# JzHuai0108/sim3opt

Measured on NVIDIA B200. Metric: Sim3 LM iterations/s, higher is better.
Workload: dtype f64

## Files before the change

sim3opt_b200/csrc/amg.cu:

```cuda
#include <algorithm>
#include <cstdlib>
#include <functional>

#include <cooperative_groups.h>

#include "amg.h"
#include "comm.h"
#include "problem.h"
#include "reduce.cuh"
#include "sim3_math.cuh"

namespace s3o {

namespace {

#define DD (D * D)
constexpr int NREL = 13;
constexpr int kCoarsestMax = 16;
constexpr int kCoarsestMaxBig = 128;
constexpr int kBigGraph = 20000;
constexpr int kMaxLevels = 12;
constexpr double kOmega = 0.7;

struct LevelDev {
// ... 1523 lines not shown
        auto kgrid = [](int n) { int g = (n + 15) / 16; return g > 148 * 8 ? 148 * 8 : (g < 1 ? 1 : g); };
        std::function<void(int)> solve;
        auto cycle = [&](int l, const double *rin, double *xout) {
            LevelDev &L = st->lev[l];
            LevelDev &C = st->lev[l + 1];
            amg_row_kernel<D, 0><<<rows(L.n), 128, 0, s>>>(L.n, L.rowptr, L.colidx, L.A, L.Dinv, rin, nullptr, L.x, kOmega, sc, chk);
            amg_row_kernel<D, 1><<<rows(L.n), 128, 0, s>>>(L.n, L.rowptr, L.colidx, L.A, L.Dinv, rin, L.x, L.t, kOmega, sc, chk);
            amg_restrict_kernel<D><<<(C.n + 15) / 16, 128, 0, s>>>(C.n, C.mem_ptr, C.mem_idx, C.rel, C.pad_fine, L.t, C.r, sc, chk);
            launches += 3;
            trace_mark(p, "lev: sweep+residual+restrict");
            solve(l + 1);
            amg_prolong_kernel<D><<<(L.n + 127) / 128, 128, 0, s>>>(L.n, C.agg, C.rel, C.pad_fine, C.x2, L.x, sc, chk);
            amg_row_kernel<D, 2><<<rows(L.n), 128, 0, s>>>(L.n, L.rowptr, L.colidx, L.A, L.Dinv, rin, L.x, xout, kOmega, sc, chk);
            launches += 2;
            trace_mark(p, "lev: prolong+sweep");
        };
        solve = [&](int l) {
            LevelDev &L = st->lev[l];
            if (l >= st->coop_first) {
                CoopParams P{};
                P.nlev = nl - l;
                P.dense = st->dense ? 1 : 0;
                P.N = st->lev.back().n * D;
                P.inv = st->d_dense;
                P.kdepth = nk > l ? nk - l : 0;
                P.kmask = st->kmask >> l;
                P.dots = st->d_cdots;
                static long long *d_dbg = nullptr;
                static int dbg_calls = 0;
                static const bool dbg_on = getenv("S3O_COOP_DBG") != nullptr;
                if (dbg_on && !d_dbg) { cudaMalloc(&d_dbg, 128 * sizeof(long long)); }
                const bool dbg_now = dbg_on && ++dbg_calls == 200;
                if (dbg_now) { cudaMemsetAsync(d_dbg, 0, 128 * sizeof(long long), s); P.dbg = d_dbg; }
                for (int k = l; k < nl; ++k) {
                    LevelDev &S = st->lev[k];
                    CoopLevel &T = P.lev[k - l];
                    T.n = S.n; T.pad_fine = S.pad_fine;
                    T.rowptr = S.rowptr; T.colidx = S.colidx; T.mem_ptr = S.mem_ptr; T.mem_idx = S.mem_idx; T.agg = S.agg;
                    T.A = S.A; T.Dinv = S.Dinv; T.rel = S.rel; T.r = S.r; T.x = S.x; T.x2 = S.x2; T.t = S.t;
                    T.z1 = S.z1; T.q1 = S.q1; T.rp = S.rp; T.z2 = S.z2; T.acol = S.acol;
                }
                double omega = kOmega;
                int chk_ = chk;
                GridBarrier gb{};
                void *args[] = { &P, &omega, (void *)&sc, &chk_, &gb };
                int grid = (L.n * 8 + kCoopThreads - 1) / kCoopThreads;
                grid = std::max(8, std::min(grid, st->coop_grid));
                for (int k = 0; k < P.nlev; ++k) {
                    const long long lanes = (long long)grid * kCoopThreads, n = P.lev[k].n;
                    P.lev[k].G = n * 32 <= lanes ? 4 : (n * 16 <= lanes ? 2 : 1);
                }
                if (launch_persistent(p, (const void *)amg_coop_kernel<D>, grid, kCoopThreads, args, 5)) rc_inner = S3O_ERR_CUDA;
                ++launches;
                trace_mark(p, "cooperative kernel");
                if (dbg_now) {
                    long long h[128];
                    cudaStreamSynchronize(s);
                    cudaMemcpy(h, d_dbg, sizeof h, cudaMemcpyDeviceToHost);
                    int khz = 1; cudaDeviceGetAttribute(&khz, cudaDevAttrClockRate, p->device);
                    fprintf(stderr, "S3O_COOP_DBG: phase times of one cooperative-kernel call (us, SM clock %d kHz)\n ", khz);
                    for (int q = 1; q < 120 && h[q]; ++q) fprintf(stderr, " %d:%.1f", q, (double)(h[q] - h[q - 1]) / khz * 1e3);
                    fprintf(stderr, "\n");
                }
                return;
            }
            if ((st->kmask >> l) & 1u) {
                KScal *ks = st->d_ks + l;
                const int n = L.n * D;
                cycle(l, L.r, L.z1);
                amg_kdots_kernel<D, 128><<<kgrid(L.n), 128, 0, s>>>(L.n, L.rowptr, L.colidx, L.A, L.z1, L.r, nullptr, L.q1, p->d_partials, ks, 0, p->d_sc, chk);
                amg_kaxpy_kernel<<<std::min((n + 255) / 256, 148 * 8), 256, 0, s>>>(n, L.r, L.q1, L.rp, ks, 0, sc, chk);
                trace_mark(p, "lev: kdots+axpy");
                cycle(l, L.rp, L.z2);
                amg_kdots_kernel<D, 128><<<kgrid(L.n), 128, 0, s>>>(L.n, L.rowptr, L.colidx, L.A, L.z2, L.rp, L.q1, nullptr, p->d_partials, ks, 1, p->d_sc, chk);
                amg_kaxpy_kernel<<<std::min((n + 255) / 256, 148 * 8), 256, 0, s>>>(n, L.z1, L.z2, L.x2, ks, 1, sc, chk);
                launches += 4;
                trace_mark(p, "lev: kdots+combine");
            } else {
                cycle(l, L.r, L.x2);
            }
        };
        solve(0);
        if (rc_inner) { set_error("multilevel K-cycle: persistent-kernel launch failed: %s", s3o_last_error()); return rc_inner; }
        std::swap(st->lev[0].x, st->lev[0].x2);
    } else {
        for (int l = 0; l < lt; ++l) {
            LevelDev &L = st->lev[l];
            LevelDev &C = st->lev[l + 1];
            amg_row_kernel<D, 0><<<rows(L.n), 128, 0, s>>>(L.n, L.rowptr, L.colidx, L.A, L.Dinv, L.r, nullptr, L.x, kOmega, sc, chk);
            amg_row_kernel<D, 1><<<rows(L.n), 128, 0, s>>>(L.n, L.rowptr, L.colidx, L.A, L.Dinv, L.r, L.x, L.t, kOmega, sc, chk);
            amg_restrict_kernel<D><<<(C.n + 15) / 16, 128, 0, s>>>(C.n, C.mem_ptr, C.mem_idx, C.rel, C.pad_fine, L.t, C.r, sc, chk);
            launches += 3;
        }
        {
            TailParams P{};
            P.nlev = nl - lt;
            P.dense = st->dense ? 1 : 0;
            P.N = st->lev.back().n * D;
            P.inv = st->d_dense;
            for (int l = lt; l < nl; ++l) {
                LevelDev &L = st->lev[l];
                TailLevel &T = P.lev[l - lt];
                T.n = L.n; T.pad_fine = L.pad_fine;
                T.rowptr = L.rowptr; T.colidx = L.colidx; T.mem_ptr = L.mem_ptr; T.mem_idx = L.mem_idx; T.agg = L.agg;
                T.A = L.A; T.Dinv = L.Dinv; T.rel = L.rel; T.r = L.r; T.x = L.x; T.x2 = L.x2; T.t = L.t;
            }
            amg_tail_kernel<D><<<kTailCtas, kTailThreads, 0, s>>>(P, kOmega, sc, chk);
            for (int l = lt; l < nl; ++l) std::swap(st->lev[l].x, st->lev[l].x2);
            ++launches;
        }
        for (int l = lt - 1; l >= 0; --l) {
            LevelDev &L = st->lev[l];
            LevelDev &C = st->lev[l + 1];
            amg_prolong_kernel<D><<<(L.n + 127) / 128, 128, 0, s>>>(L.n, C.agg, C.rel, C.pad_fine, C.x, L.x, sc, chk);
            amg_row_kernel<D, 2><<<rows(L.n), 128, 0, s>>>(L.n, L.rowptr, L.colidx, L.A, L.Dinv, L.r, L.x, L.x2, kOmega, sc, chk);
            std::swap(L.x, L.x2);
            launches += 2;
        }
    }
    {
        LevelDev &L = st->lev[0];
        constexpr int NT = 256;
        const int rows = st->dist ? st->n_own : L.n_fine;
        int grid = (rows + NT - 1) / NT;
        if (grid > 148 * 8) grid = 148 * 8;
        if (grid < 1) grid = 1;
        int dgrid = (L.n * D + NT - 1) / NT;
        if (dgrid > 148) dgrid = 148;
        if (dgrid < 1) dgrid = 1;
        amg_coarse_dot_kernel<NT><<<dgrid, NT, 0, s>>>(L.n * D, L.r, L.x, p->d_partials, p->d_sc, init, tol, max_iter);
        amg_prolong0_kernel<D, NT><<<grid, NT, 0, s>>>(rows, L.agg, L.rel, L.pad_fine, L.x, p->d_z, p->d_p, sc, init);
        launches += 2;
        trace_mark(p, "coarse dot + fine prolong");
    }
    return check_launch(p, launches);
}

}

#define S3O_AMG_DISPATCH(CALL7, CALL4, CALL1)                  \
    switch (p->kind) {                                         \
    case S3O_KIND_SIM3: return CALL7;                          \
    case S3O_KIND_SCALE_TRANS: return CALL4;                   \
    case S3O_KIND_SCALE: return CALL1;                         \
    default: set_error("multilevel preconditioner: pose-graph problems only"); return S3O_ERR_UNSUPPORTED; \
    }
int amg_update_frames(s3o_problem *p) {
    S3O_AMG_DISPATCH((update_frames_t<7, S3O_KIND_SIM3>(p)), (update_frames_t<4, S3O_KIND_SCALE_TRANS>(p)),
                     (update_frames_t<1, S3O_KIND_SCALE>(p)))
}
int amg_update_values(s3o_problem *p, double lambda) {
    S3O_AMG_DISPATCH((update_values_t<7, S3O_KIND_SIM3>(p, lambda)), (update_values_t<4, S3O_KIND_SCALE_TRANS>(p, lambda)),
                     (update_values_t<1, S3O_KIND_SCALE>(p, lambda)))
}
int amg_apply(s3o_problem *p, int init, double tol, int max_iter) {
    S3O_AMG_DISPATCH(apply_t<7>(p, init, tol, max_iter), apply_t<4>(p, init, tol, max_iter), apply_t<1>(p, init, tol, max_iter))
}
#undef S3O_AMG_DISPATCH

void amg_counts(const s3o_problem *p, int64_t *rebuilds, int64_t *reuses) {
    if (!rebuilds || !reuses) { if (p->amg) p->amg->rebuilds = p->amg->reuses = 0; return; }
    *rebuilds = p->amg ? p->amg->rebuilds : 0;
    *reuses = p->amg ? p->amg->reuses : 0;
}
void amg_set_counts(s3o_problem *p, int64_t rebuilds, int64_t reuses) {
    if (p->amg) { p->amg->rebuilds = rebuilds; p->amg->reuses = reuses; }
}
void amg_invalidate_frames(s3o_problem *p) { if (p->amg) { p->amg->frames_valid = false; p->amg->lin_changed = true; } }

}
```

sim3opt_b200/csrc/kernels.cuh:

```cuda
#pragma once
#include <cuda_runtime.h>
#include <stdint.h>

namespace s3o {

struct DevScalars {
    double rz;
    double rz_new;
    double rr;
    double pq;
    double alpha, beta;
    double rr0;
    double tol2;
    double chi2;
    double scale;
    double maxdiag;
    double xmax;
    int done;
    int iters, max_iter;
    int precond_fail;
    int halo_fail;
    unsigned counters[8];
};

struct GraphDev {
    int kind, d, est_dim, ninfo;
    int nv, nv_pad, ne, ne_pad, nf, nb;
    const double *est;
    const double *aux;
    const int32_t *hidx;
    const int32_t *sv0, *sv1;
    const double *meas;
    const double *info;
    bool info_diag;
    int robust_kind;
    double robust_param;
    bool math_corrected;
    int model_flags;
    const uint8_t *primary;
    const int32_t *ghidx;
};

struct StructDev {
    const int32_t *rowptr, *colidx, *blk_row;
    const int32_t *blk_ebeg, *blk_eend;
    const int32_t *blk_src;
    const int32_t *multi_blk;
    int n_multi;
    const int32_t *colT_ptr, *colT_blk;
    const int32_t *inc_ptr, *inc_ent;
    const int32_t *e_blk;
    const int32_t *tile_row;
    int ntiles;
    int n_own;
    double *const *ghost_src;
};

constexpr int kMaxPartials = 4096;

void launch_pack_vertices(const double *aos, int n, int n_pad, int dim, double *soa, cudaStream_t st);
void launch_unpack_vertices(const double *soa, int n, int n_pad, int dim, double *aos, cudaStream_t st);
void launch_pack_edges(const double *meas_aos, const double *info_aos, const int32_t *perm, int ne, int ne_pad,
                       int est_dim, int d, int info_diag, double *meas, double *info, cudaStream_t st);

void launch_chi2(const GraphDev &g, double *partials, DevScalars *sc, cudaStream_t st);
void launch_edge_errors(const GraphDev &g, double *err_sorted , double *chi2_sorted ,
                        cudaStream_t st);
void launch_linearize(const GraphDev &g, int jac_mode, double h, double *scratch , const int32_t *e_blk,
                      const int32_t *blk_src, double *Hdirect, cudaStream_t st);
int scratch_stride(int d);
void launch_assemble(const GraphDev &g, const StructDev &s, const double *scratch, double *H, double *b,
                     cudaStream_t st);
void launch_retract(const GraphDev &g, const double *x, double *est_out, cudaStream_t st);

void launch_maxdiag(int d, const double *H, const int32_t *rowptr, int nf, double *partials, DevScalars *sc,
                    cudaStream_t st);
void launch_pcg_fin_init(DevScalars *sc, double tol, int max_iter, cudaStream_t st);
void launch_pcg_fin_spmv(DevScalars *sc, cudaStream_t st);
void launch_pcg_fin_update(DevScalars *sc, cudaStream_t st);
void launch_pack_rows(int d, const double *vec, const int32_t *idx, int n, double *out, const DevScalars *sc,
                      cudaStream_t st);
void launch_precond(int d, const double *H, const int32_t *rowptr, int nf, double lambda, double *Minv,
                    DevScalars *sc, cudaStream_t st);
void launch_spmv(int d, const double *H, const StructDev &s, int nf, double lambda, const double *p, double *q1,
                 double *T, double *partials, DevScalars *sc, int pcg_mode, cudaStream_t st);
void launch_finish_q(int d, const StructDev &s, int nf, const double *q1, const double *T, double *q, cudaStream_t st);
void launch_pcg_init(int d, int nf, const double *b, const double *Minv, double *x, double *r, double *z, double *p,
                     double *partials, DevScalars *sc, double tol, int max_iter, int dist, cudaStream_t st);
void launch_pcg_update(int d, const StructDev &s, int nf, const double *q1, const double *T, const double *Minv,
                       const double *p, double *x, double *r, double *z, double *partials, DevScalars *sc,
                       int dist, cudaStream_t st);
void launch_pcg_pupdate(int d, int nf, const double *z, double *p, const DevScalars *sc, cudaStream_t st);
void launch_scale(int n, const double *x, const double *b, double lambda, double *partials, DevScalars *sc,
                  cudaStream_t st);
int launches_per_pcg_iter();
void launch_halo_signal(long long *own_flag, long long epoch, cudaStream_t st);
void launch_halo_wait(long long *const *peer_flags, int n_peers, long long epoch, DevScalars *sc, cudaStream_t st);
void launch_scale_vec(int n, const double *in, double s, double *out, cudaStream_t st);
void launch_fill_const(int n, double v, double *out, cudaStream_t st);
void launch_fill_alternating(int n, double *out, cudaStream_t st);
int spmv_tile_blocks(int d);
int spmv2_configure();
int spmv3_tile_blocks(int d);
void launch_spmv3(int d, const double *H, const StructDev &s, int nf, double lambda, const double *p, double *q1,
// ... 10 lines not shown
```

sim3opt_b200/csrc/problem.cu:

```cuda
#include <algorithm>
#include <cfloat>
#include <cmath>
#include <cstdarg>
#include <cstdio>
#include <cstring>
#include <cstdlib>
#include <memory>
#include <thread>
#include <vector>

#include "problem.h"
#include "amg.h"
#include "direct.h"

namespace s3o {

static thread_local char g_err[512] = "";
void set_error(const char *fmt, ...) {
    va_list ap;
    va_start(ap, fmt);
    vsnprintf(g_err, sizeof g_err, fmt, ap);
    va_end(ap);
}

// ... 139 lines not shown
        launch_spmv2(p->d, p->d_H, s, own_rows(p), lambda, x, p->d_q1, p->d_T, p->d_partials, p->d_sc, pcg_mode,
                     p->dist, p->stream);
}

int do_chi2(s3o_problem *p, int which) {
    if (p->kind == S3O_KIND_BA) return ba_chi2(p, which);
    if (p->S.ne_act == 0) {
        S3O_CUDA(cudaMemsetAsync(&p->d_sc->chi2, 0, sizeof(double), p->stream));
        return allreduce_sum(p, &p->d_sc->chi2, 1);
    }
    launch_chi2(graph_view(p, which), p->d_partials, p->d_sc, p->stream);
    int rc = check_launch(p, 1);
    return rc ? rc : allreduce_sum(p, &p->d_sc->chi2, 1);
}

int do_linearize(s3o_problem *p) {
    if (p->kind == S3O_KIND_BA) return ba_linearize(p);
    const GraphDev g = graph_view(p, p->cur);
    launch_linearize(g, p->jac_mode, p->jac_h, p->d_scratch, p->d_e_blk, p->d_blk_src, p->d_H, p->stream);
    launch_assemble(g, struct_view(p), p->d_scratch, p->d_H, p->d_b, p->stream);
    amg_invalidate_frames(p);
    direct_invalidate(p);
    p->linearized = true;
    return check_launch(p, 2);
}

}

namespace s3o {
bool wants_multilevel(const s3o_problem *p) {
    const int nf = p->dist ? p->plan.nf_global : p->S.nf;
    return p->kind != S3O_KIND_BA && p->kind != 100  &&
           p->scale_model == S3O_SCALE_MODEL_DIFFERENCE &&
           (p->precond == S3O_PRECOND_MULTILEVEL || (p->precond == S3O_PRECOND_AUTO && (nf >= 20000 || p->auto_multilevel)));
}

int do_solve(s3o_problem *p, double lambda, int *status, int *iters, double *rel_res, bool defer_sync) {
    if (p->linsolver != S3O_LINSOLVER_PCG) {
        int rcd = p->dist ? S3O_OK : direct_setup(p);
        if (rcd) return rcd;
        if (direct_available(p)) {
            if ((rcd = direct_solve(p, lambda, p->reuse_factor))) return rcd;
            if (status) *status = 0;
            if (iters) *iters = 0;
            if (rel_res) *rel_res = 0;
            if (defer_sync) return S3O_OK;
            if ((rcd = sync_scalars(p))) return rcd;
            if (status) *status = p->h_sc->done;
            return S3O_OK;
        }
        if (p->linsolver == S3O_LINSOLVER_DIRECT) {
            set_error("s3o_set_linear_solver(DIRECT): %s", p->dist ? "not available in the partitioned solve"
                                                                   : "the factor of this graph is too large; use PCG");
            return S3O_ERR_UNSUPPORTED;
        }
    }
    bool amg = false;
    int rc;
    if (wants_multilevel(p)) {
        if ((rc = amg_setup(p))) return rc;
        amg = amg_levels(p) > 0;
    }
    if ((rc = pcg_prepare(p, lambda, amg))) return rc;
    if ((rc = pcg_iterate(p, lambda, amg, p->pcg_tol, p->pcg_max_iter))) return rc;
    if (p->precond == S3O_PRECOND_AUTO && (p->kind == S3O_KIND_SIM3 || p->kind == S3O_KIND_SCALE_TRANS)) {
        if (!amg && p->h_sc->iters > 256) p->auto_multilevel = true;
        else if (amg && p->auto_multilevel && p->h_sc->iters <= 8) p->auto_multilevel = false;
    }
    if (status) *status = p->h_sc->done ? p->h_sc->done : 2;
    if (iters) *iters = p->h_sc->iters;
    if (rel_res) *rel_res = p->h_sc->rr0 > 0 ? std::sqrt(p->h_sc->rr / p->h_sc->rr0) : 0.0;
    return S3O_OK;
}

void hessian_product(s3o_problem *p, const double *x) { run_spmv(p, struct_view(p), 0.0, x, 0); }

int pcg_prepare(s3o_problem *p, double lambda, bool amg) {
    launch_precond(p->d, p->d_H, p->d_rowptr, own_rows(p), lambda, p->d_Minv, p->d_sc, p->stream);
    int rc = check_launch(p, 1);
    if (!rc && amg) rc = amg_update_values(p, lambda);
    return rc;
}

int pcg_iterate(s3o_problem *p, double lambda, bool amg, double tol, int max_iter) {
    const int nf = own_rows(p), d = p->d;
    const int dist = p->dist ? 1 : 0;
    const StructDev s = struct_view(p);
    const PartitionPlan &P = p->plan;
    auto halo = [&]() -> int {
        if (!dist) return S3O_OK;
        if (p->p2p) {
            ++p->halo_epoch;
            launch_halo_signal(p->d_flag, p->halo_epoch, p->stream);
            launch_halo_wait(p->d_peer_flags, p->n_peers, p->halo_epoch, p->d_sc, p->stream);
            p->stats.kernel_launches += 2;
            return S3O_OK;
        }
        launch_pack_rows(d, p->d_p, p->d_send_idx, (int)P.send_idx.size(), p->d_sendbuf, p->d_sc, p->stream);
        p->stats.kernel_launches += 1;
        if (comm_halo(p->comm, p->d_sendbuf, P.send_off.data(), P.send_count.data(), p->d_p + (size_t)P.n_own * d,
                      P.recv_off.data(), P.recv_count.data(), d, p->stream)) {
            set_error("%s", comm_last_error());
            return S3O_ERR_NCCL;
        }
        return S3O_OK;
    };
    int rc;
    const int defer = dist || amg;
    launch_pcg_init(d, nf, p->d_b, p->d_Minv, p->d_x, p->d_r, p->d_z, p->d_p, p->d_partials, p->d_sc, tol,
                    max_iter, defer, p->stream);
    rc = check_launch(p, 1);
    if (rc) return rc;
    if (amg) {
        if ((rc = amg_apply(p, 1, tol, max_iter))) return rc;
    } else if (dist) {
        if ((rc = allreduce_sum(p, &p->d_sc->rz_new, 2))) return rc;
        launch_pcg_fin_init(p->d_sc, tol, max_iter, p->stream);
        p->stats.kernel_launches += 1;
    }
    int batch = p->last_pcg_iters > 0 ? std::max(2, std::min(64, p->last_pcg_iters - 1)) : 8, launched = 0;
    if (p->trace_state == 1 && p->trace_solve > 0) --p->trace_solve;
    for (;;) {
        for (int k = 0; k < batch; ++k) {
            const bool sample = ((launched + k) & 15) == 7 && p->spmv_ev_used < s3o_problem::kSpmvEvents;
            if (p->trace_state == 1 && p->trace_solve == 0 && launched + k == 4) { p->trace_state = 2; trace_mark(p, "start"); }
            if ((rc = halo())) return rc;
            if (sample) {
                p->spmv_ev_iter[p->spmv_ev_used] = launched + k;
                cudaEventRecord(p->spmv_ev[2 * p->spmv_ev_used], p->stream);
            }
            run_spmv(p, s, lambda, p->d_p, 1);
            trace_mark(p, "spmv");
            if (sample) cudaEventRecord(p->spmv_ev[2 * p->spmv_ev_used++ + 1], p->stream);
            if (dist) {
                if ((rc = allreduce_sum(p, &p->d_sc->pq, 1))) return rc;
                launch_pcg_fin_spmv(p->d_sc, p->stream);
            }
            launch_pcg_update(d, s, nf, p->d_q1, p->d_T, p->d_Minv, p->d_p, p->d_x, p->d_r, p->d_z, p->d_partials,
                              p->d_sc, defer, p->stream);
            trace_mark(p, "pcg_update");
            if (amg) {
                if ((rc = amg_apply(p, 0, tol, max_iter))) return rc;
                if (p->trace_state == 2) { trace_mark(p, "end"); p->trace_state = 3; }
                continue;
            }
            if (dist) {
                if ((rc = allreduce_sum(p, &p->d_sc->rz_new, 2))) return rc;
                launch_pcg_fin_update(p->d_sc, p->stream);
            }
            launch_pcg_pupdate(d, nf, p->d_z, p->d_p, p->d_sc, p->stream);
        }
        launched += batch;
        rc = check_launch(p, (amg ? (dist ? 3 : 2) : (dist ? 5 : 3)) * batch);
        if (rc) return rc;
        rc = sync_scalars(p);
        if (rc) return rc;
        if (p->trace_state == 3) {
            float tot = 0;
            cudaEventElapsedTime(&tot, p->trace.front().second, p->trace.back().second);
            fprintf(stderr, "S3O_TRACE one PCG iteration: %.1f us\n", tot * 1e3f);
            for (size_t t = 1; t < p->trace.size(); ++t) {
                float ms = 0;
                cudaEventElapsedTime(&ms, p->trace[t - 1].second, p->trace[t].second);
                fprintf(stderr, "  %-28s %8.1f us\n", p->trace[t].first, ms * 1e3f);
            }
            for (auto &t : p->trace) cudaEventDestroy(t.second);
            p->trace.clear();
            p->trace_state = 0;
        }
        for (int e = 0; e < p->spmv_ev_used; ++e) {
            float ms = 0;
            if (cudaEventElapsedTime(&ms, p->spmv_ev[2 * e], p->spmv_ev[2 * e + 1]) == cudaSuccess &&
                (!p->h_sc->done || p->spmv_ev_iter[e] < p->h_sc->iters)) {
                p->stats.ms_spmv_sampled += ms;
                p->stats.n_spmv_sampled += 1;
            }
        }
        p->spmv_ev_used = 0;
        if (p->h_sc->done || launched >= max_iter + batch) break;
        batch = launched < 16 ? std::max(2, launched / 2) : std::min(64, launched);
    }
    p->stats.pcg_iterations += p->h_sc->iters;
    p->last_pcg_iters = p->h_sc->iters;
    if (p->h_sc->done != 1) p->stats.pcg_unconverged += 1;
    return S3O_OK;
}
}

namespace s3o {

int upload_structure_arrays(s3o_problem *p, int rows_own, bool on_device) {
    HostStructure &S = p->S;
    int rc = 0;
    if (!on_device) {
        std::vector<int32_t> blk_row(S.nb);
        for (int r = 0; r < S.nf; ++r)
            for (int k = S.rowptr[r]; k < S.rowptr[r + 1]; ++k) blk_row[k] = r;
        rc = rc ? rc : upload(p, &p->d_rowptr, S.rowptr);
        rc = rc ? rc : upload(p, &p->d_colidx, S.colidx);
        rc = rc ? rc : upload(p, &p->d_blk_row, blk_row);
        rc = rc ? rc : upload(p, &p->d_colT_ptr, S.colT_ptr);
        rc = rc ? rc : upload(p, &p->d_colT_blk, S.colT_blk);
    }
    S.max_row_blocks = 0;
    for (int r = 0; r < rows_own; ++r) S.max_row_blocks = std::max(S.max_row_blocks, S.rowptr[r + 1] - S.rowptr[r]);
    S.tile_blocks = (p->spmv_version == 4 && p->d == 7) ? spmv4_tile_blocks(p->spmv4_cfg)
                    : (p->spmv_version >= 3 ? spmv3_tile_blocks(p->d) : spmv_tile_blocks(p->d));
    build_tiles(S.rowptr, rows_own, S.tile_blocks, S.tile_row);
    rc = rc ? rc : upload(p, &p->d_tile_row, S.tile_row);
    return rc;
}

int alloc_linear_system(s3o_problem *p) {
    const HostStructure &S = p->S;
    const size_t nfd = (size_t)std::max(S.nf, p->dist ? p->plan.seg : 0) * p->d, dd = (size_t)p->d * p->d;
    int rc = 0;
    rc = rc ? rc : dev_alloc(&p->d_H, (size_t)S.nb * dd + 2);
    rc = rc ? rc : dev_alloc(&p->d_b, nfd);
    rc = rc ? rc : dev_alloc(&p->d_x, nfd);
    rc = rc ? rc : dev_alloc(&p->d_r, nfd);
    rc = rc ? rc : dev_alloc(&p->d_z, nfd);
    rc = rc ? rc : dev_alloc(&p->d_p, nfd);
    rc = rc ? rc : dev_alloc(&p->d_q1, nfd);
    rc = rc ? rc : dev_alloc(&p->d_T, (size_t)S.nb * p->d);
    rc = rc ? rc : dev_alloc(&p->d_Minv, (size_t)S.nf * dd);
    return rc;
}

}

namespace {
int setup_p2p(s3o_problem *p) {
    p->want_p2p_setup = false;
    if (getenv("S3O_NO_P2P") || !uses_spmv4(p)) return S3O_OK;
    const PartitionPlan &P = p->plan;
    const int world = P.world, rank = P.rank, d = p->d;
    struct Handles { cudaIpcMemHandle_t vec, flag; };
    int rc = dev_alloc(&p->d_flag, 1);
    if (rc) return rc;
    S3O_CUDA(cudaMemsetAsync(p->d_flag, 0, sizeof(long long), p->stream));
    Handles mine{};
    int ok = cudaIpcGetMemHandle(&mine.vec, p->d_p) == cudaSuccess && cudaIpcGetMemHandle(&mine.flag, p->d_flag) == cudaSuccess;
    cudaGetLastError();
    unsigned char *d_h = nullptr;
    if ((rc = dev_alloc(&d_h, sizeof(Handles) * (size_t)(world + 1)))) return rc;
    S3O_CUDA(cudaMemcpyAsync(d_h + sizeof(Handles) * world, &mine, sizeof(Handles), cudaMemcpyHostToDevice, p->stream));
    if (comm_allgather_bytes(p->comm, d_h + sizeof(Handles) * world, d_h, sizeof(Handles), p->stream)) {
        cudaFree(d_h); set_error("%s", comm_last_error()); return S3O_ERR_NCCL;
    }
    std::vector<Handles> all(world);
    S3O_CUDA(cudaMemcpyAsync(all.data(), d_h, sizeof(Handles) * world, cudaMemcpyDeviceToHost, p->stream));
    S3O_CUDA(cudaStreamSynchronize(p->stream));
    cudaFree(d_h);
    std::vector<double *> peer_vec(world, nullptr);
    std::vector<long long *> flags;
    for (int q = 0; q < world && ok; ++q) {
        if (q == rank || P.recv_count[q] == 0) continue;
        void *v = nullptr, *f = nullptr;
        if (cudaIpcOpenMemHandle(&v, all[q].vec, cudaIpcMemLazyEnablePeerAccess) != cudaSuccess) { ok = 0; break; }
        p->ipc_mapped.push_back(v);
        if (cudaIpcOpenMemHandle(&f, all[q].flag, cudaIpcMemLazyEnablePeerAccess) != cudaSuccess) { ok = 0; break; }
        p->ipc_mapped.push_back(f);
        peer_vec[q] = (double *)v;
// ... 3 lines not shown
    if (flags.size() > 32) ok = 0;
    double *d_ok = nullptr;
    if ((rc = dev_alloc(&d_ok, 1))) return rc;
    const double fail = ok ? 0.0 : 1.0;
    S3O_CUDA(cudaMemcpyAsync(d_ok, &fail, sizeof(double), cudaMemcpyHostToDevice, p->stream));
    if (comm_allreduce_max(p->comm, d_ok, 1, p->stream)) { cudaFree(d_ok); set_error("%s", comm_last_error()); return S3O_ERR_NCCL; }
    double any_fail = 1;
    S3O_CUDA(cudaMemcpyAsync(&any_fail, d_ok, sizeof(double), cudaMemcpyDeviceToHost, p->stream));
    S3O_CUDA(cudaStreamSynchronize(p->stream));
    cudaFree(d_ok);
    if (any_fail != 0.0) { close_p2p(p); return S3O_OK; }
    std::vector<double *> src(P.n_ghost);
    for (int t = 0; t < P.n_ghost; ++t) {
        const int gidx = P.ghosts[t], q = gidx / P.seg;
        src[t] = peer_vec[q] + (size_t)(gidx - q * P.seg) * d;
    }
    rc = upload(p, &p->d_ghost_src, src);
    rc = rc ? rc : upload(p, &p->d_peer_flags, flags);
    if (rc) return rc;
    S3O_CUDA(cudaStreamSynchronize(p->stream));
    p->n_peers = (int)flags.size();
    p->halo_epoch = 0;
    p->p2p = true;
    return S3O_OK;
}
}

extern "C" {

const char *s3o_last_error(void) { return g_err; }
int s3o_version(void) { return 100; }

int s3o_device_count(void) {
    int n = 0;
    if (cudaGetDeviceCount(&n) != cudaSuccess) { cudaGetLastError(); return 0; }
    return n;
}

static constexpr int kKindLinear = 100;

static int create_impl(int kind, int linear_dim, int device, s3o_problem **out) {
    if (!out) { set_error("s3o_create: out is NULL"); return S3O_ERR_INVALID; }
    *out = nullptr;
    int d, est_dim;
    switch (kind) {
    case kKindLinear: d = linear_dim; est_dim = 0; break;
    case S3O_KIND_SIM3: d = 7; est_dim = 8; break;
    case S3O_KIND_SCALE_TRANS: d = 4; est_dim = 4; break;
    case S3O_KIND_SCALE: d = 1; est_dim = 1; break;
    case S3O_KIND_BA: d = 6; est_dim = 7; break;
    default: set_error("s3o_create: unsupported kind %d", kind); return S3O_ERR_UNSUPPORTED;
    }
    int ndev = 0;
    if (cudaGetDeviceCount(&ndev) != cudaSuccess || ndev == 0) {
        cudaGetLastError();
        set_error("s3o_create: no CUDA device available (this library has no CPU path)");
        return S3O_ERR_CUDA;
    }
    if (device < 0 || device >= ndev) { set_error("s3o_create: device %d out of range (%d devices)", device, ndev); return S3O_ERR_INVALID; }
    S3O_CUDA(cudaSetDevice(device));
    s3o_problem *p = new s3o_problem();
    p->kind = kind; p->d = d; p->est_dim = est_dim; p->ninfo = d * (d + 1) / 2; p->device = device;
    cudaError_t e = cudaStreamCreateWithFlags(&p->stream, cudaStreamNonBlocking);
    if (e != cudaSuccess) { set_error("cudaStreamCreate: %s", cudaGetErrorString(e)); delete p; return S3O_ERR_CUDA; }
    p->own_stream = true;
    if (spmv2_configure() != 0) { set_error("s3o_create: cannot configure SpMV shared memory"); delete p; return S3O_ERR_CUDA; }
    if (const char *v = getenv("S3O_TRACE")) { p->trace_state = atoi(v) > 0 ? 1 : 0; p->trace_solve = atoi(v); }
    if (const char *v = getenv("S3O_SPMV_VERSION")) p->spmv_version = atoi(v);
    if (const char *v = getenv("S3O_SPMV_GRID")) {
        const int g = atoi(v);
        if (g >= 1 && g <= kMaxPartials) p->spmv_grid_cap = g;
    }
    if (const char *v = getenv("S3O_SPMV4_CFG")) {
        const int c = atoi(v);
        if (c >= 0 && c <= 2) p->spmv4_cfg = c;
    }
    if (const char *v = getenv("S3O_PRECOND")) {
        const int k = atoi(v);
        if (k >= S3O_PRECOND_AUTO && k <= S3O_PRECOND_MULTILEVEL && (k != S3O_PRECOND_MULTILEVEL || kind != S3O_KIND_BA)) p->precond = k;
    }
    for (auto &ev : p->ev) cudaEventCreate(&ev);
    for (auto &ev : p->spmv_ev) cudaEventCreate(&ev);
    if (const char *v = getenv("S3O_COOP_LAUNCH")) p->coop_launch = atoi(v) != 0;
    if (dev_alloc(&p->d_sc, 1) || dev_alloc(&p->d_partials, 3 * kMaxPartials) || dev_alloc(&p->d_gridbar, 2) ||
        cudaMallocHost((void **)&p->h_sc, sizeof(DevScalars)) != cudaSuccess) {
        s3o_destroy(p);
        return S3O_ERR_CUDA;
    }
    cudaMemsetAsync(p->d_sc, 0, sizeof(DevScalars), p->stream);
    cudaMemsetAsync(p->d_gridbar, 0, 2 * sizeof(unsigned), p->stream);
    memset(p->h_sc, 0, sizeof(DevScalars));
    p->stats.dim = d;
    *out = p;
    return S3O_OK;
}

int s3o_create(int kind, int device, s3o_problem **out) {
    if (kind == kKindLinear) { set_error("s3o_create: unsupported kind %d", kind); return S3O_ERR_UNSUPPORTED; }
    return create_impl(kind, 0, device, out);
}

int s3o_linsolver_create(int device, int block_dim, s3o_linsolver **out) {
    if (block_dim != 1 && block_dim != 4 && block_dim != 6 && block_dim != 7) {
        set_error("s3o_linsolver_create: block dimension %d (supported: 1, 4, 6, 7)", block_dim);
        return S3O_ERR_UNSUPPORTED;
    }
    return create_impl(kKindLinear, block_dim, device, out);
}

int s3o_linsolver_destroy(s3o_linsolver *p) { return s3o_destroy(p); }

int s3o_linsolver_solve(s3o_linsolver *p, int n, const int32_t *colptr, const int32_t *rowidx, const double *blocks,
                        int column_major, double lambda, const double *b, double *x, int *method, int *pcg_iterations) {
    if (!p || p->kind != kKindLinear || n < 0 || !colptr || (n > 0 && (!rowidx || !blocks || !b || !x))) { set_error("s3o_linsolver_solve: bad arguments"); return S3O_ERR_INVALID; }
    if (n == 0) return S3O_OK;
    cudaSetDevice(p->device);
    const int d = p->d, dd = d * d, nb = colptr[n];
    bool same = p->built && p->S.nf == n && p->S.nb == nb &&
                memcmp(p->S.ccs_colptr.data(), colptr, sizeof(int32_t) * (n + 1)) == 0 &&
                memcmp(p->S.ccs_rowidx.data(), rowidx, sizeof(int32_t) * nb) == 0;
    if (!same) {
        free_structure(p);
        std::vector<int32_t> v0, v1;
        for (int c = 0; c < n; ++c) {
            bool diag = false;
            for (int k = colptr[c]; k < colptr[c + 1]; ++k) {
                const int r = rowidx[k];
                if (r < 0 || r > c || (k > colptr[c] && r <= rowidx[k - 1])) {
                    set_error("s3o_linsolver_solve: column %d is not an upper block-CCS column (rows ascending, row <= column)", c);
                    return S3O_ERR_INVALID;
                }
                if (r == c) diag = true;
                else { v0.push_back(r); v1.push_back(c); }
            }
            if (!diag) { set_error("s3o_linsolver_solve: column %d has no diagonal block", c); return S3O_ERR_INVALID; }
        }
        p->nv = n;
        p->fixed.assign(n, 0);
        build_structure_host(n, nullptr, (int)v0.size(), v0.data(), v1.data(), p->S);
        if (p->S.nb != nb || memcmp(p->S.ccs_rowidx.data(), rowidx, sizeof(int32_t) * nb) != 0) { set_error("s3o_linsolver_solve: pattern mismatch"); return S3O_ERR_INVALID; }
        int rc = upload_structure_arrays(p, n);
        rc = rc ? rc : alloc_linear_system(p);
        if (rc) { free_structure(p); return rc; }
        p->built = true;
        p->stats.n_free = n; p->stats.n_blocks = nb;
    }
    std::vector<double> H((size_t)nb * dd);
    for (int c = 0; c < nb; ++c) {
        double *dst = H.data() + (size_t)p->S.ccs2bsr[c] * dd;
        const double *src = blocks + (size_t)c * dd;
        if (!column_major) memcpy(dst, src, sizeof(double) * dd);
        else
            for (int r = 0; r < d; ++r)
                for (int cc = 0; cc < d; ++cc) dst[r * d + cc] = src[cc * d + r];
    }
    S3O_CUDA(cudaMemcpyAsync(p->d_H, H.data(), H.size() * sizeof(double), cudaMemcpyHostToDevice, p->stream));
    S3O_CUDA(cudaMemcpyAsync(p->d_b, b, (size_t)n * d * sizeof(double), cudaMemcpyHostToDevice, p->stream));
    p->stats.h2d_bytes += (int64_t)((H.size() + (size_t)n * d) * sizeof(double));
    p->linearized = true;
    direct_invalidate(p);
    int status = 0, iters = 0;
    int rc = do_solve(p, lambda, &status, &iters, nullptr);
    if (rc) return rc;
    S3O_CUDA(cudaMemcpyAsync(x, p->d_x, (size_t)n * d * sizeof(double), cudaMemcpyDeviceToHost, p->stream));
    S3O_CUDA(cudaStreamSynchronize(p->stream));
    p->stats.d2h_bytes += (int64_t)n * d * 8;
    if (method) *method = direct_available(p) && p->linsolver != S3O_LINSOLVER_PCG ? S3O_LINSOLVER_DIRECT : S3O_LINSOLVER_PCG;
    if (pcg_iterations) *pcg_iterations = iters;
    if (status == 3) { set_error("s3o_linsolver_solve: the matrix is not positive definite (pivot / PCG breakdown)"); return S3O_ERR_SOLVE; }
    if (status == 2) { set_error("s3o_linsolver_solve: PCG hit the iteration cap"); return S3O_ERR_SOLVE; }
    return S3O_OK;
}

int s3o_destroy(s3o_problem *p) {
    if (!p) return S3O_OK;
    cudaSetDevice(p->device);
    if (p->stream) cudaStreamSynchronize(p->stream);
    free_structure(p);
    ba_destroy(p);
    dev_free(p->d_meas_aos); dev_free(p->d_info_aos);
    dev_free(p->d_est[0]); dev_free(p->d_est[1]); dev_free(p->d_aux);
    dev_free(p->d_sc); dev_free(p->d_partials); dev_free(p->d_gridbar);
    comm_destroy(p->comm);
    if (p->h_sc) cudaFreeHost(p->h_sc);
    for (auto &ev : p->ev) if (ev) cudaEventDestroy(ev);
    for (auto &ev : p->spmv_ev) if (ev) cudaEventDestroy(ev);
    dev_free(p->d_est_snap);
    dev_free(p->d_stage);
    if (p->own_stream && p->stream) cudaStreamDestroy(p->stream);
    delete p;
    return S3O_OK;
}

int s3o_comm_unique_id(char *id128) {
    if (!id128) return S3O_ERR_INVALID;
    if (comm_unique_id(id128)) { set_error("%s", comm_last_error()); return S3O_ERR_NCCL; }
    return S3O_OK;
}

int s3o_set_comm(s3o_problem *p, int rank, int world, const char *id128) {
    if (!p || world < 1 || rank < 0 || rank >= world || (world > 1 && !id128)) { set_error("s3o_set_comm: bad arguments"); return S3O_ERR_INVALID; }
    if (p->kind == S3O_KIND_BA && world > 1) {
        set_error("s3o_set_comm: bundle adjustment has no partitioned path (replicas only, SURVEY.md 8e)");
        return S3O_ERR_UNSUPPORTED;
    }
    cudaSetDevice(p->device);
    free_structure(p);
    comm_destroy(p->comm);
    p->dist = false;
    if (world == 1) return S3O_OK;
    if (comm_init(p->comm, rank, world, id128)) { set_error("%s", comm_last_error()); return S3O_ERR_NCCL; }
    p->dist = true;
    return S3O_OK;
}

int s3o_set_stream(s3o_problem *p, void *cuda_stream) {
    if (!p) return S3O_ERR_INVALID;
    cudaSetDevice(p->device);
    if (p->stream) cudaStreamSynchronize(p->stream);
    if (p->own_stream && p->stream) cudaStreamDestroy(p->stream);
    p->own_stream = false;
    p->stream = (cudaStream_t)cuda_stream;
    if (!cuda_stream) {
        S3O_CUDA(cudaStreamCreateWithFlags(&p->stream, cudaStreamNonBlocking));
        p->own_stream = true;
    }
    return S3O_OK;
}

static int ensure_stage(s3o_problem *p) {
    if (p->d_stage) return S3O_OK;
    return dev_alloc(&p->d_stage, (size_t)p->nv * p->est_dim);
}

static int upload_estimates(s3o_problem *p, const double *est) {
    const size_t cnt = (size_t)p->nv * p->est_dim;
    int rc = ensure_stage(p);
    if (rc) return rc;
    double *tmp = p->d_stage;
    cudaError_t e = cudaMemcpyAsync(tmp, est, cnt * sizeof(double), cudaMemcpyHostToDevice, p->stream);
    if (e == cudaSuccess) {
        launch_pack_vertices(tmp, p->nv, p->nv_pad, p->est_dim, p->d_est[p->cur], p->stream);
        e = cudaStreamSynchronize(p->stream);
    }
    if (e != cudaSuccess) { set_error("upload_estimates: %s", cudaGetErrorString(e)); return S3O_ERR_CUDA; }
    p->stats.h2d_bytes += (int64_t)(cnt * sizeof(double));
    p->stats.kernel_launches += 1;
    return S3O_OK;
}

int s3o_set_vertices(s3o_problem *p, int n, const double *est, const uint8_t *fixed, const double *aux) {
    if (!p || n < 0 || (n > 0 && !est)) { set_error("s3o_set_vertices: bad arguments"); return S3O_ERR_INVALID; }
    if (p->kind == S3O_KIND_BA) { set_error("s3o_set_vertices: a BA problem takes s3o_ba_set_cameras / s3o_ba_set_points"); return S3O_ERR_INVALID; }
    if (p->kind == S3O_KIND_SCALE_TRANS && !aux && n > 0) { set_error("s3o_set_vertices: SCALE_TRANS needs aux rotations"); return S3O_ERR_INVALID; }
    cudaSetDevice(p->device);
    free_structure(p);
    dev_free(p->d_est[0]); dev_free(p->d_est[1]); dev_free(p->d_aux);
    p->nv = n;
    p->nv_pad = pad32(n);
    p->cur = 0;
    p->lm_valid = false;
    dev_free(p->d_est_snap);
// ... 1010 lines not shown
```

sim3opt_b200/csrc/problem.h:

```cpp
#pragma once
#include <chrono>
#include <cstdio>
#include <cstdlib>
#include <vector>

#include "comm.h"
#include "internal.h"
#include "kernels.cuh"
#include "gridbar.cuh"

namespace s3o {

template <class T>
int dev_alloc(T **ptr, size_t count) {
    *ptr = nullptr;
    if (count == 0) count = 1;
    S3O_CUDA(cudaMalloc((void **)ptr, count * sizeof(T)));
    return S3O_OK;
}
template <class T>
void dev_free(T *&ptr) {
    if (ptr) cudaFree(ptr);
    ptr = nullptr;
}
// ... 7 lines not shown

using s3o::Comm;
using s3o::DevScalars;
using s3o::HostStructure;
using s3o::PartitionPlan;

struct s3o_problem {
    int kind = 0, d = 0, est_dim = 0, ninfo = 0, device = 0;
    cudaStream_t stream = nullptr;
    bool own_stream = false;
    int nv = 0, ne = 0;
    std::vector<uint8_t> fixed;
    std::vector<int32_t> v0, v1;
    bool has_info = false, has_aux = false, info_diag = false;
    double *d_meas_aos = nullptr, *d_info_aos = nullptr;
    int nv_pad = 0, ne_pad = 0;
    double *d_est[2] = { nullptr, nullptr };
    int cur = 0;
    double *d_aux = nullptr;
    int32_t *d_hidx = nullptr, *d_sv0 = nullptr, *d_sv1 = nullptr;
    double *d_meas = nullptr, *d_info = nullptr;
    HostStructure S;
    bool built = false;
    int32_t *d_rowptr = nullptr, *d_colidx = nullptr, *d_blk_row = nullptr, *d_blk_ebeg = nullptr, *d_blk_eend = nullptr;
    int32_t *d_colT_ptr = nullptr, *d_colT_blk = nullptr, *d_inc_ptr = nullptr, *d_inc_ent = nullptr, *d_e_blk = nullptr;
    int32_t *d_tile_row = nullptr;
    int32_t *d_blk_src = nullptr, *d_multi_blk = nullptr;
    Comm comm;
    bool dist = false;
    PartitionPlan plan;
    int user_ne = 0;
    std::vector<int32_t> gv0, gv1;
    int32_t *d_ghidx = nullptr, *d_send_idx = nullptr;
    uint8_t *d_primary = nullptr;
    double *d_sendbuf = nullptr, *d_xg = nullptr;
    bool p2p = false, want_p2p_setup = false;
    long long halo_epoch = 0;
    long long *d_flag = nullptr;
    double **d_ghost_src = nullptr;
    long long **d_peer_flags = nullptr;
    int n_peers = 0;
    std::vector<void *> ipc_mapped;
    int spmv_version = 4;
    int spmv_grid_cap = 148 * 2;
    int spmv4_cfg = 0;
    double *d_H = nullptr, *d_b = nullptr, *d_x = nullptr, *d_r = nullptr, *d_z = nullptr, *d_p = nullptr;
    double *d_q1 = nullptr, *d_T = nullptr, *d_Minv = nullptr, *d_scratch = nullptr, *d_partials = nullptr;
    DevScalars *d_sc = nullptr, *h_sc = nullptr;
    unsigned *d_gridbar = nullptr;
    bool coop_launch = false;
    int robust_kind = S3O_ROBUST_NONE;
    double robust_param = 0;
    int math_mode = S3O_MATH_REFERENCE;
    int scale_model = S3O_SCALE_MODEL_DIFFERENCE;
    int jac_mode = S3O_JAC_ANALYTIC;
    double jac_h = 1e-9;
    double tau = 1e-5, user_lambda = 0;
    int max_trials = 10;
    double stop_step = 0, stop_pred = 0;
    double pcg_tol = 1e-8;
    int pcg_max_iter = 1000;
    int last_pcg_iters = 0;
    int precond = S3O_PRECOND_AUTO;
    bool auto_multilevel = false;
    bool linearized = false;
    int lm_resume = 0;
    bool lm_valid = false;
    double lm_lambda = 0, lm_ni = 2, lm_chi = 0;
    double lm_prev_step = 0, lm_est_dist = 0;
    int lm_stop_hits = 0;
    double *d_est_snap = nullptr;
    double *d_stage = nullptr;
    static constexpr int kSpmvEvents = 64;
    cudaEvent_t spmv_ev[2 * kSpmvEvents] = {};
    int spmv_ev_used = 0;
    int spmv_ev_iter[kSpmvEvents] = {};
    s3o_stats stats{};
    cudaEvent_t ev[8] = {};
    s3o::BaState *ba = nullptr;
    s3o::AmgState *amg = nullptr;
    s3o::DirectState *direct = nullptr;
    int linsolver = S3O_LINSOLVER_AUTO;
    bool reuse_factor = false;
    std::vector<std::pair<const char *, cudaEvent_t>> trace;
    int trace_state = 0, trace_solve = 0;
};

namespace s3o {

template <class T>
int upload(s3o_problem *p, T **dst, const std::vector<T> &src) {
    int rc = dev_alloc(dst, src.size());
    if (rc) return rc;
    if (!src.empty()) {
        S3O_CUDA(cudaMemcpyAsync(*dst, src.data(), src.size() * sizeof(T), cudaMemcpyHostToDevice, p->stream));
        p->stats.h2d_bytes += (int64_t)(src.size() * sizeof(T));
    }
    return S3O_OK;
}

StructDev struct_view(const s3o_problem *p);
void free_structure(s3o_problem *p);
void close_p2p(s3o_problem *p);
int check_launch(s3o_problem *p, int n);
int sync_scalars(s3o_problem *p);
int upload_structure_arrays(s3o_problem *p, int rows_own, bool on_device = false);
int alloc_linear_system(s3o_problem *p);
int do_solve(s3o_problem *p, double lambda, int *status, int *iters, double *rel_res, bool defer_sync = false);
int pcg_prepare(s3o_problem *p, double lambda, bool amg);
int pcg_iterate(s3o_problem *p, double lambda, bool amg, double tol, int max_iter);
void hessian_product(s3o_problem *p, const double *x);

int direct_setup(s3o_problem *p);
bool direct_available(const s3o_problem *p);
int direct_solve(s3o_problem *p, double lambda, bool reuse_factor);
void direct_invalidate(s3o_problem *p);
void direct_destroy(s3o_problem *p);
int direct_marginals(s3o_problem *p, int n_pairs, const int32_t *rows, const int32_t *cols, double *out, cudaEvent_t *ev);
struct MarginalsRun {
    DirectState *S = nullptr;
    const DirectPlan *plan = nullptr;
    uint64_t serial = 0;
    const double *Sig = nullptr;
    const double *out = nullptr;
    const int *fail = nullptr;
};
int marginals_open(s3o_problem *p, const char *who, int n_pairs, const int32_t *rows, const int32_t *cols, MarginalsRun *run);
int marginals_factor(s3o_problem *p, const MarginalsRun &run, cudaEvent_t *ev);
int marginals_pick(s3o_problem *p, const MarginalsRun &run, int n_pairs);
int marginals_iterative(s3o_problem *p, bool *iterative);
int pcg_marginals(s3o_problem *p, int n_pairs, const int32_t *rows, const int32_t *cols, double *out, cudaEvent_t *ev);
inline int launch_persistent(s3o_problem *p, const void *func, int grid, int block, void **args, int nargs, size_t smem = 0) {
    GridBarrier *gb = (GridBarrier *)args[nargs - 1];
    gb->counter = p->d_gridbar;
    gb->abort = (int *)(p->d_gridbar + 1);
    gb->cooperative = p->coop_launch ? 1 : 0;
    if (p->coop_launch) {
        S3O_CUDA(cudaLaunchCooperativeKernel(func, dim3(grid), dim3(block), args, smem, p->stream));
        return S3O_OK;
    }
    S3O_CUDA(cudaMemsetAsync(p->d_gridbar, 0, sizeof(unsigned), p->stream));
    S3O_CUDA(cudaLaunchKernel(func, dim3(grid), dim3(block), args, smem, p->stream));
    return S3O_OK;
}
inline void trace_mark(s3o_problem *p, const char *what) {
    if (p->trace_state != 2) return;
    cudaEvent_t e;
    cudaEventCreate(&e);
    cudaEventRecord(e, p->stream);
    p->trace.push_back({ what, e });
}

bool wants_multilevel(const s3o_problem *p);
int amg_setup(s3o_problem *p);
void amg_destroy(s3o_problem *p);
int amg_levels(const s3o_problem *p);
void amg_counts(const s3o_problem *p, int64_t *rebuilds, int64_t *reuses);
void amg_invalidate_frames(s3o_problem *p);
int amg_update_frames(s3o_problem *p);
int amg_update_values(s3o_problem *p, double lambda);
int amg_apply(s3o_problem *p, int init, double tol, int max_iter);
void amg_set_counts(s3o_problem *p, int64_t rebuilds, int64_t reuses);

void ba_destroy(s3o_problem *p);
int ba_build_structure(s3o_problem *p);
int ba_chi2(s3o_problem *p, int which);
int ba_linearize(s3o_problem *p);
int ba_max_diag(s3o_problem *p);
int ba_solve(s3o_problem *p, double lambda, int *status, int *iters, double *rel_res);
int ba_retract_and_scale(s3o_problem *p, double lambda, int trial);
int ba_upload_step(s3o_problem *p, const double *x);
int ba_download_step(s3o_problem *p, double *x);
int ba_snapshot(s3o_problem *p, int restore);

}
```

Baseline: 49.05.

## Run PCG iterations inside a CUDA graph while-loop conditional node

Result: faster. 50.11 (median of 6 runs) (+2.2%).

```diff
diff --git a/sim3opt_b200/csrc/amg.cu b/sim3opt_b200/csrc/amg.cu
--- a/sim3opt_b200/csrc/amg.cu
+++ b/sim3opt_b200/csrc/amg.cu
@@ -1629,7 +1629,6 @@
         };
         solve(0);
         if (rc_inner) { set_error("multilevel K-cycle: persistent-kernel launch failed: %s", s3o_last_error()); return rc_inner; }
-        std::swap(st->lev[0].x, st->lev[0].x2);
     } else {
         for (int l = 0; l < lt; ++l) {
             LevelDev &L = st->lev[l];
@@ -1653,15 +1652,13 @@
                 T.A = L.A; T.Dinv = L.Dinv; T.rel = L.rel; T.r = L.r; T.x = L.x; T.x2 = L.x2; T.t = L.t;
             }
             amg_tail_kernel<D><<<kTailCtas, kTailThreads, 0, s>>>(P, kOmega, sc, chk);
-            for (int l = lt; l < nl; ++l) std::swap(st->lev[l].x, st->lev[l].x2);
             ++launches;
         }
         for (int l = lt - 1; l >= 0; --l) {
             LevelDev &L = st->lev[l];
             LevelDev &C = st->lev[l + 1];
-            amg_prolong_kernel<D><<<(L.n + 127) / 128, 128, 0, s>>>(L.n, C.agg, C.rel, C.pad_fine, C.x, L.x, sc, chk);
+            amg_prolong_kernel<D><<<(L.n + 127) / 128, 128, 0, s>>>(L.n, C.agg, C.rel, C.pad_fine, C.x2, L.x, sc, chk);
             amg_row_kernel<D, 2><<<rows(L.n), 128, 0, s>>>(L.n, L.rowptr, L.colidx, L.A, L.Dinv, L.r, L.x, L.x2, kOmega, sc, chk);
-            std::swap(L.x, L.x2);
             launches += 2;
         }
     }
@@ -1675,8 +1672,8 @@
         int dgrid = (L.n * D + NT - 1) / NT;
         if (dgrid > 148) dgrid = 148;
         if (dgrid < 1) dgrid = 1;
-        amg_coarse_dot_kernel<NT><<<dgrid, NT, 0, s>>>(L.n * D, L.r, L.x, p->d_partials, p->d_sc, init, tol, max_iter);
-        amg_prolong0_kernel<D, NT><<<grid, NT, 0, s>>>(rows, L.agg, L.rel, L.pad_fine, L.x, p->d_z, p->d_p, sc, init);
+        amg_coarse_dot_kernel<NT><<<dgrid, NT, 0, s>>>(L.n * D, L.r, L.x2, p->d_partials, p->d_sc, init, tol, max_iter);
+        amg_prolong0_kernel<D, NT><<<grid, NT, 0, s>>>(rows, L.agg, L.rel, L.pad_fine, L.x2, p->d_z, p->d_p, sc, init);
         launches += 2;
         trace_mark(p, "coarse dot + fine prolong");
     }
diff --git a/sim3opt_b200/csrc/kernels.cuh b/sim3opt_b200/csrc/kernels.cuh
--- a/sim3opt_b200/csrc/kernels.cuh
+++ b/sim3opt_b200/csrc/kernels.cuh
@@ -20,6 +20,7 @@
     int iters, max_iter;
     int precond_fail;
     int halo_fail;
+    int loop_iters;
     unsigned counters[8];
 };
 
diff --git a/sim3opt_b200/csrc/problem.cu b/sim3opt_b200/csrc/problem.cu
--- a/sim3opt_b200/csrc/problem.cu
+++ b/sim3opt_b200/csrc/problem.cu
@@ -245,6 +245,74 @@
     return rc;
 }
 
+__global__ void pcg_loop_cond_kernel(cudaGraphConditionalHandle h, DevScalars *sc, const unsigned *gridbar, int body) {
+    sc->loop_iters = body ? sc->loop_iters + 1 : 0;
+    cudaGraphSetConditional(h, sc->done == 0 && gridbar[1] == 0 ? 1u : 0u);
+}
+
+template <class Iteration>
+int pcg_graph_launch(s3o_problem *p, Iteration &&iteration, int *per_iter) {
+    if (!p->pcg_g) {
+        S3O_CUDA(cudaStreamCreateWithFlags(&p->cap_stream, cudaStreamNonBlocking));
+        S3O_CUDA(cudaGraphCreate(&p->pcg_g, 0));
+        S3O_CUDA(cudaGraphConditionalHandleCreate(&p->pcg_cond, p->pcg_g, 0, 0));
+        DevScalars *sc = p->d_sc;
+        const unsigned *bar = p->d_gridbar;
+        int body = 0;
+        void *args[] = { &p->pcg_cond, &sc, &bar, &body };
+        cudaKernelNodeParams kp{};
+        kp.func = (void *)pcg_loop_cond_kernel;
+        kp.gridDim = dim3(1);
+        kp.blockDim = dim3(1);
+        kp.kernelParams = args;
+        cudaGraphNode_t first, loop;
+        S3O_CUDA(cudaGraphAddKernelNode(&first, p->pcg_g, nullptr, 0, &kp));
+        cudaGraphNodeParams cp{};
+        cp.type = cudaGraphNodeTypeConditional;
+        cp.conditional.handle = p->pcg_cond;
+        cp.conditional.type = cudaGraphCondTypeWhile;
+        cp.conditional.size = 1;
+        S3O_CUDA(cudaGraphAddNode(&loop, p->pcg_g, &first, 1, &cp));
+        p->pcg_body = cp.conditional.phGraph_out[0];
+    }
+    size_t n = 0;
+    S3O_CUDA(cudaGraphGetNodes(p->pcg_body, nullptr, &n));
+    std::vector<cudaGraphNode_t> old(n);
+    if (n) S3O_CUDA(cudaGraphGetNodes(p->pcg_body, old.data(), &n));
+    for (cudaGraphNode_t v : old) S3O_CUDA(cudaGraphDestroyNode(v));
+    const cudaStream_t stream = p->stream;
+    const int64_t launches = p->stats.kernel_launches;
+    S3O_CUDA(cudaStreamBeginCaptureToGraph(p->cap_stream, p->pcg_body, nullptr, nullptr, 0, cudaStreamCaptureModeRelaxed));
+    p->stream = p->cap_stream;
+    int rc = iteration();
+    if (!rc) pcg_loop_cond_kernel<<<1, 1, 0, p->cap_stream>>>(p->pcg_cond, p->d_sc, p->d_gridbar, 1);
+    p->stream = stream;
+    cudaGraph_t captured = nullptr;
+    const cudaError_t e = cudaStreamEndCapture(p->cap_stream, &captured);
+    if (rc) return rc;
+    if (e != cudaSuccess) { set_error("PCG graph capture: %s", cudaGetErrorString(e)); return S3O_ERR_CUDA; }
+    *per_iter = (int)(p->stats.kernel_launches - launches) + 1;
+    p->stats.kernel_launches = launches;
+    if (p->pcg_exec) {
+        cudaGraphExecUpdateResultInfo info{};
+        if (cudaGraphExecUpdate(p->pcg_exec, p->pcg_g, &info) != cudaSuccess) {
+            cudaGetLastError();
+            cudaGraphExecDestroy(p->pcg_exec);
+            p->pcg_exec = nullptr;
+        }
+    }
+    if (!p->pcg_exec) S3O_CUDA(cudaGraphInstantiate(&p->pcg_exec, p->pcg_g, 0));
+    S3O_CUDA(cudaGraphLaunch(p->pcg_exec, stream));
+    return S3O_OK;
+}
+
+void pcg_graph_destroy(s3o_problem *p) {
+    if (p->pcg_exec) cudaGraphExecDestroy(p->pcg_exec);
+    if (p->pcg_g) cudaGraphDestroy(p->pcg_g);
+    if (p->cap_stream) cudaStreamDestroy(p->cap_stream);
+    p->pcg_exec = nullptr; p->pcg_g = nullptr; p->pcg_body = nullptr; p->cap_stream = nullptr;
+}
+
 int pcg_iterate(s3o_problem *p, double lambda, bool amg, double tol, int max_iter) {
     const int nf = own_rows(p), d = p->d;
     const int dist = p->dist ? 1 : 0;
@@ -281,56 +349,39 @@
         launch_pcg_fin_init(p->d_sc, tol, max_iter, p->stream);
         p->stats.kernel_launches += 1;
     }
-    int batch = p->last_pcg_iters > 0 ? std::max(2, std::min(64, p->last_pcg_iters - 1)) : 8, launched = 0;
-    if (p->trace_state == 1 && p->trace_solve > 0) --p->trace_solve;
-    for (;;) {
-        for (int k = 0; k < batch; ++k) {
-            const bool sample = ((launched + k) & 15) == 7 && p->spmv_ev_used < s3o_problem::kSpmvEvents;
-            if (p->trace_state == 1 && p->trace_solve == 0 && launched + k == 4) { p->trace_state = 2; trace_mark(p, "start"); }
-            if ((rc = halo())) return rc;
-            if (sample) {
-                p->spmv_ev_iter[p->spmv_ev_used] = launched + k;
-                cudaEventRecord(p->spmv_ev[2 * p->spmv_ev_used], p->stream);
-            }
-            run_spmv(p, s, lambda, p->d_p, 1);
-            trace_mark(p, "spmv");
-            if (sample) cudaEventRecord(p->spmv_ev[2 * p->spmv_ev_used++ + 1], p->stream);
-            if (dist) {
-                if ((rc = allreduce_sum(p, &p->d_sc->pq, 1))) return rc;
-                launch_pcg_fin_spmv(p->d_sc, p->stream);
-            }
-            launch_pcg_update(d, s, nf, p->d_q1, p->d_T, p->d_Minv, p->d_p, p->d_x, p->d_r, p->d_z, p->d_partials,
-                              p->d_sc, defer, p->stream);
-            trace_mark(p, "pcg_update");
-            if (amg) {
-                if ((rc = amg_apply(p, 0, tol, max_iter))) return rc;
-                if (p->trace_state == 2) { trace_mark(p, "end"); p->trace_state = 3; }
-                continue;
-            }
-            if (dist) {
-                if ((rc = allreduce_sum(p, &p->d_sc->rz_new, 2))) return rc;
-                launch_pcg_fin_update(p->d_sc, p->stream);
-            }
-            launch_pcg_pupdate(d, nf, p->d_z, p->d_p, p->d_sc, p->stream);
-        }
-        launched += batch;
-        rc = check_launch(p, (amg ? (dist ? 3 : 2) : (dist ? 5 : 3)) * batch);
-        if (rc) return rc;
-        rc = sync_scalars(p);
-        if (rc) return rc;
-        if (p->trace_state == 3) {
-            float tot = 0;
-            cudaEventElapsedTime(&tot, p->trace.front().second, p->trace.back().second);
-            fprintf(stderr, "S3O_TRACE one PCG iteration: %.1f us\n", tot * 1e3f);
-            for (size_t t = 1; t < p->trace.size(); ++t) {
-                float ms = 0;
-                cudaEventElapsedTime(&ms, p->trace[t - 1].second, p->trace[t].second);
-                fprintf(stderr, "  %-28s %8.1f us\n", p->trace[t].first, ms * 1e3f);
-            }
-            for (auto &t : p->trace) cudaEventDestroy(t.second);
-            p->trace.clear();
-            p->trace_state = 0;
-        }
+    auto iteration = [&](int k, bool sample) -> int {
+        sample = sample && p->spmv_ev_used < s3o_problem::kSpmvEvents;
+        if (p->trace_state == 1 && p->trace_solve == 0 && k == 4) { p->trace_state = 2; trace_mark(p, "start"); }
+        int rci;
+        if ((rci = halo())) return rci;
+        if (sample) {
+            p->spmv_ev_iter[p->spmv_ev_used] = k;
+            cudaEventRecord(p->spmv_ev[2 * p->spmv_ev_used], p->stream);
+        }
+        run_spmv(p, s, lambda, p->d_p, 1);
+        trace_mark(p, "spmv");
+        if (sample) cudaEventRecord(p->spmv_ev[2 * p->spmv_ev_used++ + 1], p->stream);
+        if (dist) {
+            if ((rci = allreduce_sum(p, &p->d_sc->pq, 1))) return rci;
+            launch_pcg_fin_spmv(p->d_sc, p->stream);
+        }
+        launch_pcg_update(d, s, nf, p->d_q1, p->d_T, p->d_Minv, p->d_p, p->d_x, p->d_r, p->d_z, p->d_partials,
+                          p->d_sc, defer, p->stream);
+        trace_mark(p, "pcg_update");
+        if (amg) {
+            if ((rci = check_launch(p, dist ? 3 : 2))) return rci;
+            if ((rci = amg_apply(p, 0, tol, max_iter))) return rci;
+            if (p->trace_state == 2) { trace_mark(p, "end"); p->trace_state = 3; }
+            return S3O_OK;
+        }
+        if (dist) {
+            if ((rci = allreduce_sum(p, &p->d_sc->rz_new, 2))) return rci;
+            launch_pcg_fin_update(p->d_sc, p->stream);
+        }
+        launch_pcg_pupdate(d, nf, p->d_z, p->d_p, p->d_sc, p->stream);
+        return check_launch(p, dist ? 5 : 3);
+    };
+    auto collect_samples = [&]() {
         for (int e = 0; e < p->spmv_ev_used; ++e) {
             float ms = 0;
             if (cudaEventElapsedTime(&ms, p->spmv_ev[2 * e], p->spmv_ev[2 * e + 1]) == cudaSuccess &&
@@ -340,8 +391,40 @@
             }
         }
         p->spmv_ev_used = 0;
-        if (p->h_sc->done || launched >= max_iter + batch) break;
-        batch = launched < 16 ? std::max(2, launched / 2) : std::min(64, launched);
+    };
+    if (p->pcg_graph && !dist) {
+        if ((rc = iteration(0, true))) return rc;
+        int per_iter = 0;
+        if ((rc = pcg_graph_launch(p, [&]() { return iteration(1, false); }, &per_iter))) return rc;
+        if ((rc = sync_scalars(p))) return rc;
+        p->stats.kernel_launches += 1 + (int64_t)per_iter * p->h_sc->loop_iters;
+        collect_samples();
+    } else {
+        int batch = p->last_pcg_iters > 0 ? std::max(2, std::min(64, p->last_pcg_iters - 1)) : 8, launched = 0;
+        if (p->trace_state == 1 && p->trace_solve > 0) --p->trace_solve;
+        for (;;) {
+            for (int k = 0; k < batch; ++k)
+                if ((rc = iteration(launched + k, ((launched + k) & 15) == 7))) return rc;
+            launched += batch;
+            rc = sync_scalars(p);
+            if (rc) return rc;
+            if (p->trace_state == 3) {
+                float tot = 0;
+                cudaEventElapsedTime(&tot, p->trace.front().second, p->trace.back().second);
+                fprintf(stderr, "S3O_TRACE one PCG iteration: %.1f us\n", tot * 1e3f);
+                for (size_t t = 1; t < p->trace.size(); ++t) {
+                    float ms = 0;
+                    cudaEventElapsedTime(&ms, p->trace[t - 1].second, p->trace[t].second);
+                    fprintf(stderr, "  %-28s %8.1f us\n", p->trace[t].first, ms * 1e3f);
+                }
+                for (auto &t : p->trace) cudaEventDestroy(t.second);
+                p->trace.clear();
+                p->trace_state = 0;
+            }
+            collect_samples();
+            if (p->h_sc->done || launched >= max_iter + batch) break;
+            batch = launched < 16 ? std::max(2, launched / 2) : std::min(64, launched);
+        }
     }
     p->stats.pcg_iterations += p->h_sc->iters;
     p->last_pcg_iters = p->h_sc->iters;
@@ -511,6 +594,8 @@
     for (auto &ev : p->ev) cudaEventCreate(&ev);
     for (auto &ev : p->spmv_ev) cudaEventCreate(&ev);
     if (const char *v = getenv("S3O_COOP_LAUNCH")) p->coop_launch = atoi(v) != 0;
+    if (const char *v = getenv("S3O_PCG_GRAPH")) p->pcg_graph = atoi(v) != 0;
+    if (p->trace_state || p->coop_launch || getenv("S3O_COOP_DBG")) p->pcg_graph = false;
     if (dev_alloc(&p->d_sc, 1) || dev_alloc(&p->d_partials, 3 * kMaxPartials) || dev_alloc(&p->d_gridbar, 2) ||
         cudaMallocHost((void **)&p->h_sc, sizeof(DevScalars)) != cudaSuccess) {
         s3o_destroy(p);
@@ -607,6 +692,7 @@
     if (p->stream) cudaStreamSynchronize(p->stream);
     free_structure(p);
     ba_destroy(p);
+    pcg_graph_destroy(p);
     dev_free(p->d_meas_aos); dev_free(p->d_info_aos);
     dev_free(p->d_est[0]); dev_free(p->d_est[1]); dev_free(p->d_aux);
     dev_free(p->d_sc); dev_free(p->d_partials); dev_free(p->d_gridbar);
diff --git a/sim3opt_b200/csrc/problem.h b/sim3opt_b200/csrc/problem.h
--- a/sim3opt_b200/csrc/problem.h
+++ b/sim3opt_b200/csrc/problem.h
@@ -113,6 +113,12 @@
     s3o::DirectState *direct = nullptr;
     int linsolver = S3O_LINSOLVER_AUTO;
     bool reuse_factor = false;
+    bool pcg_graph = true;
+    cudaStream_t cap_stream = nullptr;
+    cudaGraph_t pcg_g = nullptr;
+    cudaGraph_t pcg_body = nullptr;
+    cudaGraphConditionalHandle pcg_cond = 0;
+    cudaGraphExec_t pcg_exec = nullptr;
     std::vector<std::pair<const char *, cudaEvent_t>> trace;
     int trace_state = 0, trace_solve = 0;
 };
@@ -140,6 +146,7 @@
 int do_solve(s3o_problem *p, double lambda, int *status, int *iters, double *rel_res, bool defer_sync = false);
 int pcg_prepare(s3o_problem *p, double lambda, bool amg);
 int pcg_iterate(s3o_problem *p, double lambda, bool amg, double tol, int max_iter);
+void pcg_graph_destroy(s3o_problem *p);
 void hessian_product(s3o_problem *p, const double *x);
 
 int direct_setup(s3o_problem *p);
```
